# drprojects/superpoint_transformer

Measured on AMD Instinct MI355X. Metric: Mpoints/s SPT fwd+bwd on S3DIS-scale NAG, higher is better.
Workload: dtype f32 (the reference's shipped matmul class - configs/train.yaml:60-61 `float32_matmul_precision: high` = TF32 / bf16x3 next to `precision: 32` - as bf16x3: matrix products on the bf16 pipe with split operands, attention and the backward of the fused layers and of the attention blocks' Linears hi*hi +

## Files before the change

### superpoint_transformer_amd/csrc/fused_pool.hip

```cpp
#include <math.h>

#include <type_traits>

#include "common.hpp"

namespace spt {
namespace fpool {

typedef float f32x4 __attribute__((ext_vector_type(4)));
typedef __bf16 bf16x8 __attribute__((ext_vector_type(8)));
typedef __bf16 bf16x4 __attribute__((ext_vector_type(4)));
typedef short s16x4 __attribute__((ext_vector_type(4)));
#ifndef SPT_FPOOL_SKIP
#define SPT_FPOOL_SKIP 0
#endif
#ifndef SPT_FPOOL_WPAD
#define SPT_FPOOL_WPAD 16
#endif
constexpr int TR = 16;
constexpr int NWF = 8;
constexpr int ARG_NONE = 0x7fffffff;

__device__ __forceinline__ double xg_sum_d(double v) {
  v += __shfl_xor(v, 16, 64);
  v += __shfl_xor(v, 32, 64);
  return v;
}
__device__ __forceinline__ float xg_sum_f(float v) {
  v += __shfl_xor(v, 16, 64);
  v += __shfl_xor(v, 32, 64);
  return v;
}
__device__ __forceinline__ void wave_sync_lds() {
  __builtin_amdgcn_fence(__ATOMIC_RELEASE, "wavefront");
  __builtin_amdgcn_wave_barrier();
  __builtin_amdgcn_fence(__ATOMIC_ACQUIRE, "wavefront");
}
template <bool B16>
__device__ __forceinline__ float4 ld4(const float* __restrict__ base, int64_t elem) {
  if constexpr (B16) {
    const uint2 u = *reinterpret_cast<const uint2*>(reinterpret_cast<const uint16_t*>(base) + elem);
    return make_float4(__uint_as_float(u.x << 16), __uint_as_float(u.x & 0xffff0000u),
                       __uint_as_float(u.y << 16), __uint_as_float(u.y & 0xffff0000u));
  } else {
    return *reinterpret_cast<const float4*>(base + elem);
  }
}
template <int NV, typename V>
__device__ __forceinline__ void split2(const float (&x)[NV], V& hi, V& lo) {
#pragma unroll
  for (int i = 0; i < NV; ++i) {
    const __bf16 h = (__bf16)x[i];
    hi[i] = h;
    lo[i] = (__bf16)(x[i] - (float)h);
  }
}
template <int NV, typename V>
__device__ __forceinline__ void split3(const float (&x)[NV], V& h, V& m, V& l) {
#pragma unroll
  for (int i = 0; i < NV; ++i) {
    const __bf16 a = (__bf16)x[i];
    const float r1 = x[i] - (float)a;
    const __bf16 b = (__bf16)r1;
    const float r2 = r1 - (float)b;
    h[i] = a;
    m[i] = b;
    l[i] = (__bf16)r2;
  }
}
__device__ __forceinline__ f32x4 mfma16(const bf16x4& a, const bf16x4& b, f32x4 c) {
  return __builtin_amdgcn_mfma_f32_16x16x16bf16_1k(__builtin_bit_cast(s16x4, a),
                                                   __builtin_bit_cast(s16x4, b), c, 0, 0, 0);
}

template <bool X16>
struct RowChunk { typedef float4 type; };
template <>
struct RowChunk<true> { typedef uint2 type; };
template <bool X16>
__device__ __forceinline__ float4 widen(const typename RowChunk<X16>::type& u) {
  if constexpr (X16) {
    return make_float4(__uint_as_float(u.x << 16), __uint_as_float(u.x & 0xffff0000u),
                       __uint_as_float(u.y << 16), __uint_as_float(u.y & 0xffff0000u));
  } else {
    return u;
  }
}
template <int K, bool X16>
__device__ __forceinline__ void load_rows(const float* __restrict__ x, int rid_l,
                                          typename RowChunk<X16>::type (&v)[TR * (K / 4) / 64], int lane) {
  constexpr int CH = K / 4, NIT = TR * CH / 64;
  static_assert(TR * CH % 64 == 0, "whole waves of chunks");
#pragma unroll
  for (int j = 0; j < NIT; ++j) {
    const int q = lane + 64 * j, rr = q / CH, k = (q - rr * CH) << 2;
    const int64_t xr = (int64_t)__shfl(rid_l, rr, 64);
    if constexpr (X16)
      v[j] = *reinterpret_cast<const uint2*>(reinterpret_cast<const uint16_t*>(x) + xr * K + k);
    else
      v[j] = *reinterpret_cast<const float4*>(x + xr * K + k);
  }
}
template <int K, int LD, bool PRE, bool X16>
__device__ __forceinline__ void store_rows(const typename RowChunk<X16>::type (&v)[TR * (K / 4) / 64],
                                           int cnt, const float* tab, float slope, float* lds, int lane) {
  constexpr int CH = K / 4, NIT = TR * CH / 64;
#pragma unroll
  for (int j = 0; j < NIT; ++j) {
    const int q = lane + 64 * j, rr = q / CH, k = (q - rr * CH) << 2;
    float4 w = widen<X16>(v[j]);
    if constexpr (PRE) {
      const float4 a = *reinterpret_cast<const float4*>(tab + k);
      const float4 s = *reinterpret_cast<const float4*>(tab + K + k);
      const float4 b = *reinterpret_cast<const float4*>(tab + 2 * K + k);
      w.x = fmaf(w.x - a.x, s.x, b.x); w.y = fmaf(w.y - a.y, s.y, b.y);
      w.z = fmaf(w.z - a.z, s.z, b.z); w.w = fmaf(w.w - a.w, s.w, b.w);
      w.x = w.x > 0.f ? w.x : w.x * slope; w.y = w.y > 0.f ? w.y : w.y * slope;
      w.z = w.z > 0.f ? w.z : w.z * slope; w.w = w.w > 0.f ? w.w : w.w * slope;
    }
    if (rr >= cnt) w = make_float4(0.f, 0.f, 0.f, 0.f);
    *reinterpret_cast<float4*>(lds + rr * LD + k) = w;
  }
}

__device__ __forceinline__ int64_t cut_at(int64_t p, int64_t r0, int64_t r1,
                                          const int32_t* __restrict__ pos_seg,
                                          const int32_t* __restrict__ rowptr) {
  if (p <= r0) return r0;
  if (p >= r1) return r1;
  const int s = __builtin_amdgcn_readfirstlane(pos_seg[p]);
  const int64_t b = (int64_t)__builtin_amdgcn_readfirstlane(rowptr[s]);
  if (b == p) return p;
  const int64_t e = (int64_t)__builtin_amdgcn_readfirstlane(rowptr[s + 1]);
  return e < r1 ? e : r1;
}

template <int K, int N, int PREC, bool IN16>
__global__ __launch_bounds__(NWF * 64, 2) void fwd_pool_kernel(
    const float* __restrict__ x, const int32_t* __restrict__ perm,
    const int32_t* __restrict__ pos_seg, const int32_t* __restrict__ rowptr,
    const float* __restrict__ W, const float* __restrict__ gnw, const float* __restrict__ pam,
    const float* __restrict__ psc, const float* __restrict__ pbs, float pslope,
    float* __restrict__ raw, int32_t* __restrict__ argpos, double* __restrict__ partial, FmlpRuns rt) {
  constexpr int KS = K / 32, KB = K / 16, NBK = N / 16, LDA = K + 4;
  constexpr int LDW = K + SPT_FPOOL_WPAD;
  static_assert(LDW % 32 == 16 || SPT_FPOOL_WPAD != 16, "conflict-free B fragments");
  constexpr int NPL = PREC == 3 ? 3 : (PREC == 2 ? 2 : 1);
  constexpr int NGB = KB * (KB + 1) / 2;
  constexpr int GLEN = K * K + K + 1;
  static_assert(K % 32 == 0 && N % 16 == 0, "shape");
  __shared__ __attribute__((aligned(16))) float a_lds[NWF][TR * LDA];
  __shared__ __attribute__((aligned(16))) float tab[4 * K];
  __shared__ __attribute__((aligned(16))) float sgn_l[N];
  __shared__ __attribute__((aligned(16))) __bf16 wpl[NPL][N * LDW];
  __shared__ double gred[K * K + K];
  const int lane = threadIdx.x & 63;
  const int wid = __builtin_amdgcn_readfirstlane(threadIdx.x >> 6);
  const int g = lane >> 4, c = lane & 15;
  const int run = blockIdx.y, gph = rt.g[run];
  const int64_t r0 = rt.r0[run], r1 = rt.r1[run];
  pam += (size_t)gph * K;
  psc += (size_t)gph * K;
  partial += ((size_t)run * gridDim.x + blockIdx.x) * GLEN;
  float* al = a_lds[wid];
  for (int i = threadIdx.x; i < K; i += NWF * 64) {
    tab[i] = pam[i];
    tab[K + i] = psc[i];
    tab[2 * K + i] = pbs[i];
    const float bsv = pbs[i];
    tab[3 * K + i] = PREC == 1 ? 0.f : (bsv > 0.f ? bsv : pslope * bsv);
  }
  for (int i = threadIdx.x; i < N; i += NWF * 64) sgn_l[i] = gnw[i] < 0.f ? -1.f : 1.f;
  for (int i = threadIdx.x; i < N * K; i += NWF * 64) {
    const int n = i / K, k = i - n * K;
    const float w = gnw[n] < 0.f ? -W[i] : W[i];
    if constexpr (PREC == 3) {
      const float w1[1] = {w};
      __bf16 a[1], b[1], cc[1];
      split3<1>(w1, a, b, cc);
      wpl[0][n * LDW + k] = a[0];
      wpl[1][n * LDW + k] = b[0];
      wpl[2][n * LDW + k] = cc[0];
    } else if constexpr (PREC == 2) {
      const __bf16 hh = (__bf16)w;
      wpl[0][n * LDW + k] = hh;
      wpl[1][n * LDW + k] = (__bf16)(w - (float)hh);
    } else {
      wpl[0][n * LDW + k] = (__bf16)w;
    }
  }
  __syncthreads();

  f32x4 GA[NGB];
#pragma unroll
  for (int i = 0; i < NGB; ++i) GA[i] = (f32x4){0.f, 0.f, 0.f, 0.f};
  float sy[KB];
#pragma unroll
  for (int kb = 0; kb < KB; ++kb) sy[kb] = 0.f;
  float pm[NBK];
  int pp[NBK];
#pragma unroll
  for (int nb = 0; nb < NBK; ++nb) {
    pm[nb] = -INFINITY;
    pp[nb] = ARG_NONE;
  }
  int cur_seg = -1;
  auto flush = [&](int seg) {
#pragma unroll
    for (int nb = 0; nb < NBK; ++nb) {
      float m = pm[nb];
      int a = pp[nb];
#pragma unroll
      for (int off = 16; off <= 32; off <<= 1) {
        const float om = __shfl_xor(m, off, 64);
        const int oa = __shfl_xor(a, off, 64);
        const bool t = (om > m) || (om == m && oa < a);
        m = t ? om : m;
        a = t ? oa : a;
      }
      if ((nb & 3) == g) {
        const size_t o = (size_t)seg * N + 16 * nb + c;
        raw[o] = m * sgn_l[16 * nb + c];
        argpos[o] = a;
      }
      pm[nb] = -INFINITY;
      pp[nb] = ARG_NONE;
    }
  };

  const int64_t nw = (int64_t)gridDim.x * NWF, w = (int64_t)blockIdx.x * NWF + wid;
  const int64_t per = (((r1 - r0 + nw - 1) / nw) + TR - 1) / TR * TR;
  const int64_t pa0 = cut_at(r0 + w * per, r0, r1, pos_seg, rowptr);
  const int64_t pb0 = (w == nw - 1) ? r1 : cut_at(r0 + (w + 1) * per, r0, r1, pos_seg, rowptr);
  const bool has_rows = pa0 < pb0;
  const int64_t plast = pb0 - 1;
  auto ids_of = [&](int64_t p, int& rid, int& sg) {
    int64_t q = p + (lane & (TR - 1));
    q = q < plast ? q : plast;
    rid = perm ? perm[q] : (int)q;
    sg = pos_seg[q];
  };
  if (has_rows) {
  int seg_a, seg_b, rid_c, seg_c;
  typename RowChunk<IN16>::type xv[TR * (K / 4) / 64];
  {
    int rid0, rid1;
    ids_of(pa0, rid0, seg_a);
    load_rows<K, IN16>(x, rid0, xv, lane);
    ids_of(pa0 + TR, rid1, seg_b);
    ids_of(pa0 + 2 * TR, rid_c, seg_c);
    wave_sync_lds();
    store_rows<K, LDA, true, IN16>(xv, (int)((pb0 - pa0) < TR ? (pb0 - pa0) : TR), tab, pslope, al, lane);
    load_rows<K, IN16>(x, rid1, xv, lane);
  }
  for (int64_t p = pa0; p < pb0; p += TR) {
    const int cnt = (int)((pb0 - p) < TR ? (pb0 - p) : TR);
    wave_sync_lds();
    f32x4 C[NBK];
#pragma unroll
    for (int nb = 0; nb < NBK; ++nb) C[nb] = (f32x4){0.f, 0.f, 0.f, 0.f};
    if constexpr (!(SPT_FPOOL_SKIP & 4)) {
      constexpr int NSTEP = KS * NBK;
      constexpr int LA = NPL == 3 ? 2 : (NPL == 2 ? 3 : 6);
      bf16x8 wf[LA + 1][NPL];
      auto ldw = [&](int step, bf16x8 (&w)[NPL]) {
        const int ks = step / NBK, nb = step - ks * NBK;
        const int wo = (16 * nb + c) * LDW + 32 * ks + 8 * g;
#pragma unroll
        for (int pl = 0; pl < NPL; ++pl) w[pl] = *reinterpret_cast<const bf16x8*>(&wpl[pl][wo]);
      };
#pragma unroll
      for (int i = 0; i < LA; ++i) ldw(i, wf[i]);
      bf16x8 x1, x2, x3;
#pragma unroll
      for (int step = 0; step < NSTEP; ++step) {
        const int ks = step / NBK, nb = step - ks * NBK;
        if (nb == 0) {
          const float4 a0 = *reinterpret_cast<const float4*>(al + c * LDA + 32 * ks + 8 * g);
          const float4 a1 = *reinterpret_cast<const float4*>(al + c * LDA + 32 * ks + 8 * g + 4);
          const float av[8] = {a0.x, a0.y, a0.z, a0.w, a1.x, a1.y, a1.z, a1.w};
          if constexpr (PREC == 3) {
            split3<8>(av, x1, x2, x3);
          } else if constexpr (PREC == 2) {
            split2<8>(av, x1, x2);
          } else {
#pragma unroll
            for (int i = 0; i < 8; ++i) x1[i] = (__bf16)av[i];
          }
        }
        if (step + LA < NSTEP) ldw(step + LA, wf[(step + LA) % (LA + 1)]);
        __builtin_amdgcn_sched_barrier(0);
        const bf16x8 (&w)[NPL] = wf[step % (LA + 1)];
        f32x4 acc = C[nb];
        if constexpr (PREC == 3) {
          acc = __builtin_amdgcn_mfma_f32_16x16x32_bf16(x3, w[0], acc, 0, 0, 0);
          acc = __builtin_amdgcn_mfma_f32_16x16x32_bf16(x1, w[NPL - 1], acc, 0, 0, 0);
          acc = __builtin_amdgcn_mfma_f32_16x16x32_bf16(x2, w[NPL > 1 ? 1 : 0], acc, 0, 0, 0);
          acc = __builtin_amdgcn_mfma_f32_16x16x32_bf16(x2, w[0], acc, 0, 0, 0);
          acc = __builtin_amdgcn_mfma_f32_16x16x32_bf16(x1, w[NPL > 1 ? 1 : 0], acc, 0, 0, 0);
        } else if constexpr (PREC == 2) {
          acc = __builtin_amdgcn_mfma_f32_16x16x32_bf16(x2, w[0], acc, 0, 0, 0);
          acc = __builtin_amdgcn_mfma_f32_16x16x32_bf16(x1, w[NPL - 1], acc, 0, 0, 0);
        }
        acc = __builtin_amdgcn_mfma_f32_16x16x32_bf16(x1, w[0], acc, 0, 0, 0);
        C[nb] = acc;
        __builtin_amdgcn_sched_barrier(0);
      }
    }
    if constexpr (!(SPT_FPOOL_SKIP & 1)) {
      bf16x4 Yh[KB], Yl[KB];
#pragma unroll
      for (int kb = 0; kb < KB; ++kb) {
        float yv[4];
#pragma unroll
        for (int r = 0; r < 4; ++r) yv[r] = al[(4 * g + r) * LDA + 16 * kb + c];
        if constexpr (PREC != 1) {
          const float sh = tab[3 * K + 16 * kb + c];
#pragma unroll
          for (int r = 0; r < 4; ++r) yv[r] = (4 * g + r < cnt) ? yv[r] - sh : 0.f;
        }
        if constexpr (PREC == 1) {
#pragma unroll
          for (int r = 0; r < 4; ++r) {
            Yh[kb][r] = (__bf16)yv[r];
            yv[r] = (float)Yh[kb][r];
          }
        } else {
          split2<4>(yv, Yh[kb], Yl[kb]);
        }
        sy[kb] += (yv[0] + yv[1]) + (yv[2] + yv[3]);
      }
      int gi = 0;
#pragma unroll
      for (int mi = 0; mi < KB; ++mi)
#pragma unroll
        for (int ni = mi; ni < KB; ++ni) {
          f32x4 acc = GA[gi];
          if constexpr (PREC != 1) {
            acc = mfma16(Yl[mi], Yl[ni], acc);
            acc = mfma16(Yl[mi], Yh[ni], acc);
            acc = mfma16(Yh[mi], Yl[ni], acc);
          }
          GA[gi] = mfma16(Yh[mi], Yh[ni], acc);
          ++gi;
        }
    }
    wave_sync_lds();
    {
      const int64_t left = pb0 - (p + TR);
      store_rows<K, LDA, true, IN16>(xv, (int)(left < 0 ? 0 : (left < TR ? left : TR)), tab, pslope, al, lane);
      asm volatile("" : "+v"(rid_c), "+v"(seg_c));
    }
    const int seg_cur = seg_a;
    if constexpr (!(SPT_FPOOL_SKIP & 2)) {
      const int pos0 = (int)p + 4 * g;
      int row = 0;
      while (row < cnt) {
        const int s = __builtin_amdgcn_readlane(seg_cur, row);
        const uint64_t diff = __ballot(lane < cnt && lane > row && seg_cur != s);
        const int e = diff ? (int)__builtin_ctzll(diff) : cnt;
        if (s != cur_seg) {
          if (cur_seg >= 0) flush(cur_seg);
          cur_seg = s;
        }
        if (row == 0 && e == TR) {
#pragma unroll
          for (int r = 0; r < 4; ++r)
#pragma unroll
            for (int nb = 0; nb < NBK; ++nb) {
              const float v = C[nb][r];
              const bool win = v > pm[nb];
              pm[nb] = win ? v : pm[nb];
              pp[nb] = win ? pos0 + r : pp[nb];
            }
        } else {
#pragma unroll
          for (int r = 0; r < 4; ++r) {
            const int rr = 4 * g + r;
            const bool in = rr >= row && rr < e;
#pragma unroll
            for (int nb = 0; nb < NBK; ++nb) {
              const float v = in ? C[nb][r] : -INFINITY;
              const bool win = v > pm[nb];
              pm[nb] = win ? v : pm[nb];
              pp[nb] = win ? pos0 + r : pp[nb];
            }
          }
        }
        row = e;
      }
    }
    load_rows<K, IN16>(x, rid_c, xv, lane);
    seg_a = seg_b;
    seg_b = seg_c;
    ids_of(p + 3 * TR, rid_c, seg_c);
  }
  }
  if (cur_seg >= 0) flush(cur_seg);

  for (int i = threadIdx.x; i < K * K + K; i += NWF * 64) gred[i] = 0.0;
  __syncthreads();
  for (int ww = 0; ww < NWF; ++ww) {
    if (wid == ww) {
      int gi = 0;
#pragma unroll
      for (int mi = 0; mi < KB; ++mi)
#pragma unroll
        for (int ni = mi; ni < KB; ++ni) {
#pragma unroll
          for (int r = 0; r < 4; ++r)
            gred[(16 * mi + 4 * g + r) * K + 16 * ni + c] += (double)GA[gi][r];
          ++gi;
        }
#pragma unroll
      for (int kb = 0; kb < KB; ++kb) {
        const double t = xg_sum_d((double)sy[kb]);
        if (g == 0) gred[K * K + 16 * kb + c] += t;
      }
    }
    __syncthreads();
  }
  const int64_t wfirst = (int64_t)blockIdx.x * NWF, wlast = wfirst + NWF - 1;
  const int64_t ba = cut_at(r0 + wfirst * per, r0, r1, pos_seg, rowptr);
  const int64_t bb = (wlast >= nw - 1) ? r1 : cut_at(r0 + (wlast + 1) * per, r0, r1, pos_seg, rowptr);
  const double nblk = (double)(bb > ba ? bb - ba : 0);
  for (int i = threadIdx.x; i < K * K; i += NWF * 64) {
    const int rr = i / K, cc = i - rr * K;
    const double gp = (rr / 16 <= cc / 16) ? gred[i] : gred[cc * K + rr];
    const double sr = (double)tab[3 * K + rr], sc_ = (double)tab[3 * K + cc];
    partial[i] = gp + sr * gred[K * K + cc] + gred[K * K + rr] * sc_ + nblk * sr * sc_;
  }
  for (int i = threadIdx.x; i < K; i += NWF * 64)
    partial[K * K + i] = gred[K * K + i] + nblk * (double)tab[3 * K + i];
  if (threadIdx.x == 0) partial[K * K + K] = (blockIdx.x == 0) ? (double)(r1 - r0) : 0.0;
}

template <int K>
__global__ __launch_bounds__(256) void gram_tables_kernel(
    const double* __restrict__ gram, const float* __restrict__ W, int N, int bfw,
    const float* __restrict__ weight, const float* __restrict__ mean_scale, float eps,
    double* __restrict__ total, float* __restrict__ mean, float* __restrict__ rstd,
    float* __restrict__ am, float* __restrict__ scale) {
  constexpr int GLEN = K * K + K + 1, CPB = 256 / K;
  __shared__ double gl[K * K + K];
  __shared__ double wl[CPB][K];
  __shared__ double r1[CPB][K], r2[CPB][K];
  const int b = blockIdx.y;
  const double* gr = gram + (size_t)b * GLEN;
  for (int i = threadIdx.x; i < K * K + K; i += 256) gl[i] = gr[i];
  const int cl = threadIdx.x / K, j = threadIdx.x - cl * K;
  const int c = blockIdx.x * CPB + cl;
  {
    float w = c < N ? W[(size_t)c * K + j] : 0.f;
    if (bfw) w = (float)(__bf16)w;
    wl[cl][j] = (double)w;
  }
  __syncthreads();
  double t = 0.0;
#pragma unroll 8
  for (int k = 0; k < K; ++k) t += gl[j * K + k] * wl[cl][k];
  r2[cl][j] = wl[cl][j] * t;
  r1[cl][j] = wl[cl][j] * gl[K * K + j];
  __syncthreads();
  for (int st = K / 2; st > 0; st >>= 1) {
    if (j < st) {
      r1[cl][j] += r1[cl][j + st];
      r2[cl][j] += r2[cl][j + st];
    }
    __syncthreads();
  }
  if (j != 0 || c >= N) return;
  double n = gr[K * K + K];
  const double nraw = n;
  if (n < 1.0) n = 1.0;
  const double s1 = r1[cl][0];
  double s2 = r2[cl][0];
  if (s2 < 0.0) s2 = 0.0;
  if (total) {
    double* tr = total + (size_t)b * (2 * N + 1);
    tr[c] = s1;
    tr[N + c] = s2;
    if (c == 0) tr[2 * N] = nraw;
  }
  const double mu = s1 / n;
  const double a = (double)mean_scale[c];
  double var = s2 / n - (2.0 * a - a * a) * mu * mu;
  if (var < 0.0) var = 0.0;
  const double rs = 1.0 / sqrt(var + (double)eps);
  const float mu32 = (float)mu, rs32 = (float)rs;
  const int o = b * N + c;
  mean[o] = mu32;
  rstd[o] = rs32;
  am[o] = (float)(a * (double)mu32);
  scale[o] = (float)((double)weight[c] * (double)rs32);
}

template <int K, bool IN16>
__global__ __launch_bounds__(256) void pool_apply_kernel(
    const int32_t* __restrict__ rowptr, const int32_t* __restrict__ perm,
    const int64_t* __restrict__ seg_graph, int64_t num_seg, int N, int64_t n_rows,
    const float* __restrict__ am, const float* __restrict__ sc, const float* __restrict__ bs,
    float slope, const float* __restrict__ gnw, const float* __restrict__ x,
    const float* __restrict__ W, const float* __restrict__ pam, const float* __restrict__ psc,
    const float* __restrict__ pbs, float pslope, int bfw, float* __restrict__ raw,
    int32_t* __restrict__ argpos, int32_t* __restrict__ arg, float* __restrict__ out) {
  const int64_t t4 = ((int64_t)blockIdx.x * blockDim.x + threadIdx.x) * 4;
  if (t4 >= num_seg * N) return;
  const int64_t s = t4 / N;
  const int c0 = (int)(t4 - s * N);
  const int a0 = rowptr[s], a1 = rowptr[s + 1];
  if (a1 <= a0) {
    const int32_t nr = (int32_t)n_rows;
    *reinterpret_cast<float4*>(out + t4) = make_float4(0.f, 0.f, 0.f, 0.f);
    *reinterpret_cast<float4*>(raw + t4) = make_float4(0.f, 0.f, 0.f, 0.f);
    if (arg) *reinterpret_cast<int4*>(arg + t4) = make_int4(nr, nr, nr, nr);
    *reinterpret_cast<int4*>(argpos + t4) = make_int4(nr, nr, nr, nr);
    return;
  }
  const int64_t gph = seg_graph ? seg_graph[s] : 0;
  const float4 h4 = *reinterpret_cast<const float4*>(raw + t4);
  const int4 p4 = *reinterpret_cast<const int4*>(argpos + t4);
  const float4 w4 = *reinterpret_cast<const float4*>(gnw + c0);
  const float4 am4 = *reinterpret_cast<const float4*>(am + gph * N + c0);
  const float4 sc4 = *reinterpret_cast<const float4*>(sc + gph * N + c0);
  const float4 bs4 = *reinterpret_cast<const float4*>(bs + c0);
  float hh[4] = {h4.x, h4.y, h4.z, h4.w};
  int pp[4] = {p4.x, p4.y, p4.z, p4.w};
  const float gw[4] = {w4.x, w4.y, w4.z, w4.w};
  const float aa[4] = {am4.x, am4.y, am4.z, am4.w}, ss[4] = {sc4.x, sc4.y, sc4.z, sc4.w};
  const float bb[4] = {bs4.x, bs4.y, bs4.z, bs4.w};
  float yy[4];
  int ar[4];
#pragma unroll
  for (int e = 0; e < 4; ++e) {
    if (gw[e] == 0.f) {
      const int c = c0 + e;
      pp[e] = a0;
      const int row = perm ? perm[a0] : a0;
      double acc = 0.0;
      for (int k = 0; k < K; ++k) {
        float v = IN16 ? __uint_as_float((unsigned)reinterpret_cast<const uint16_t*>(x)[(int64_t)row * K + k] << 16)
                       : x[(int64_t)row * K + k];
        v = fmaf(v - pam[gph * K + k], psc[gph * K + k], pbs[k]);
        v = v > 0.f ? v : v * pslope;
        float w = W[(size_t)c * K + k];
        if (bfw) {
          w = (float)(__bf16)w;
          v = (float)(__bf16)v;
        }
        acc += (double)v * (double)w;
      }
      hh[e] = (float)acc;
      raw[t4 + e] = hh[e];
      argpos[t4 + e] = pp[e];
    }
    if (arg) ar[e] = (pp[e] >= a0 && pp[e] < a1) ? (perm ? perm[pp[e]] : pp[e]) : (int32_t)n_rows;
    float y = fmaf(hh[e] - aa[e], ss[e], bb[e]);
    yy[e] = y > 0.f ? y : y * slope;
  }
  if (arg) *reinterpret_cast<int4*>(arg + t4) = make_int4(ar[0], ar[1], ar[2], ar[3]);
  *reinterpret_cast<float4*>(out + t4) = make_float4(yy[0], yy[1], yy[2], yy[3]);
}

__global__ __launch_bounds__(256) void pool_bwd_gm_kernel(
    const float* __restrict__ gout, const float* __restrict__ raw,
    const int64_t* __restrict__ seg_graph, int64_t num_seg, int N, const float* __restrict__ am,
    const float* __restrict__ sc, const float* __restrict__ bs, float slope,
    const float* __restrict__ c1, float* __restrict__ gm) {
  const int64_t t4 = ((int64_t)blockIdx.x * blockDim.x + threadIdx.x) * 4;
  if (t4 >= num_seg * N) return;
  const int64_t s = t4 / N;
  const int c = (int)(t4 - s * N);
  const int64_t gph = seg_graph ? seg_graph[s] : 0;
  const float4 go = *reinterpret_cast<const float4*>(gout + t4);
  const float4 hv = *reinterpret_cast<const float4*>(raw + t4);
  const float4 a = *reinterpret_cast<const float4*>(am + gph * N + c);
  const float4 sv = *reinterpret_cast<const float4*>(sc + gph * N + c);
  const float4 b = *reinterpret_cast<const float4*>(bs + c);
  const float4 k1 = *reinterpret_cast<const float4*>(c1 + gph * N + c);
  const float gg[4] = {go.x, go.y, go.z, go.w}, hh[4] = {hv.x, hv.y, hv.z, hv.w};
  const float aa[4] = {a.x, a.y, a.z, a.w}, ss[4] = {sv.x, sv.y, sv.z, sv.w};
  const float bb[4] = {b.x, b.y, b.z, b.w}, q1[4] = {k1.x, k1.y, k1.z, k1.w};
  float o[4];
#pragma unroll
  for (int e = 0; e < 4; ++e) {
    float g_ = gg[e];
    if (slope != 1.f) {
      const float y = fmaf(hh[e] - aa[e], ss[e], bb[e]);
      g_ = (y > 0.f) ? g_ : g_ * slope;
    }
    o[e] = q1[e] * g_;
  }
  *reinterpret_cast<float4*>(gm + t4) = make_float4(o[0], o[1], o[2], o[3]);
}

template <int K>
__global__ __launch_bounds__(256) void pool_bwd_coef_kernel(
    const float* __restrict__ W, int N, const float* __restrict__ am, const float* __restrict__ c2,
    const float* __restrict__ c3, float* __restrict__ M, float* __restrict__ c0) {
  const int b = blockIdx.x;
  extern __shared__ float sm[];
  float* Bc = sm;
  float* Ac = sm + N;
  for (int i = threadIdx.x; i < N; i += blockDim.x) {
    const float k2 = c2[b * N + i];
    Bc[i] = -k2;
    Ac[i] = fmaf(k2, am[b * N + i], -c3[b * N + i]);
  }
  __syncthreads();
  for (int i = blockIdx.y * blockDim.x + threadIdx.x; i < K * K + K; i += gridDim.y * blockDim.x) {
    double acc = 0.0;
    if (i < K * K) {
      const int j = i / K, k = i - j * K;
      for (int c = 0; c < N; ++c)
        acc += (double)W[(size_t)c * K + j] * (double)Bc[c] * (double)W[(size_t)c * K + k];
      M[(size_t)b * K * K + i] = (float)acc;
    } else {
      const int k = i - K * K;
      for (int c = 0; c < N; ++c) acc += (double)Ac[c] * (double)W[(size_t)c * K + k];
      c0[(size_t)b * K + k] = (float)acc;
    }
  }
}

template <int K>
__global__ __launch_bounds__(256) void pool_bwd_gw_dense_kernel(
    const double* __restrict__ gram, int B, const float* __restrict__ W, int N, int bfw,
    const float* __restrict__ am, const float* __restrict__ c2, const float* __restrict__ c3,
    float* __restrict__ gW) {
  constexpr int GLEN = K * K + K + 1;
  const int t = blockIdx.x * blockDim.x + threadIdx.x;
  if (t >= N * K) return;
  const int c = t / K, k = t - c * K;
  double acc = 0.0;
  for (int b = 0; b < B; ++b) {
    const double* gr = gram + (size_t)b * GLEN;
    const double k2 = (double)c2[b * N + c];
    const double Ac = (double)fmaf(c2[b * N + c], am[b * N + c], -c3[b * N + c]);
    double t1 = 0.0;
    for (int j = 0; j < K; ++j) {
      float w = W[(size_t)c * K + j];
      if (bfw) w = (float)(__bf16)w;
      t1 += (double)w * gr[j * K + k];
    }
    acc += -k2 * t1 + Ac * gr[K * K + k];
  }
  gW[t] = (float)((double)gW[t] + acc);
}

typedef __attribute__((address_space(3))) s16x4 lds_s16x4;
typedef __attribute__((address_space(3))) volatile int lds_flag_t;
__device__ __forceinline__ void flag_set(lds_flag_t* f, int v) {
  asm volatile("s_waitcnt lgkmcnt(0)" ::: "memory");
  *f = v;
}
__device__ __forceinline__ bool flag_wait(lds_flag_t* f, int v) {
  int spins = 0;
  bool ok = true;
#pragma clang loop unroll(disable)
  while (__builtin_amdgcn_readfirstlane(*f) < v) {
    __builtin_amdgcn_s_sleep(1);
    if (++spins > (1 << 22)) {
      ok = false;
      break;
    }
  }
  asm volatile("" ::: "memory");
  return ok;
}
template <int C>
__device__ __forceinline__ int pl_off(int row, int col) {
  constexpr int RPL = 128 / C;
  static_assert(C == 32 || C == 64 || C == 128, "plane row of 64, 128 or 256 bytes");
  const int swz = ((row / RPL) & (8 / RPL - 1)) << 1;
  return row * C + ((((col >> 3) ^ swz) << 3) | (col & 7));
}
__device__ __forceinline__ s16x4 tr_read(const __bf16* p) {
  return __builtin_amdgcn_ds_read_tr16_b64_v4i16((lds_s16x4*)(__attribute__((address_space(3))) void*)p);
}
template <int K, int N, bool LO, bool X16, int NW>
__global__ __launch_bounds__(NW * 64, NW / 4) void bwd_pool_kernel(
    const float* __restrict__ gm, const int32_t* __restrict__ argpos,
    const int32_t* __restrict__ perm, const int32_t* __restrict__ pos_seg,
    const float* __restrict__ xprev, const float* __restrict__ pam,
    const float* __restrict__ psc, const float* __restrict__ pbs, float pslope,
    const float* __restrict__ W, const float* __restrict__ Mg, const float* __restrict__ c0g,
    float* __restrict__ gx, float* __restrict__ gw_partial, double* __restrict__ pstat_partial,
    FmlpRuns rt) {
  constexpr int KB = K / 16, NBK = N / 16, NS = N / 32, KS = K / 32;
  constexpr int NBH = NBK / 2, KBH = KB / 2;
  constexpr int LDX = K + 4;
  constexpr int LDT = N + SPT_FPOOL_WPAD, LDM = K + SPT_FPOOL_WPAD;
  static_assert((LDT % 32 == 16 && LDM % 32 == 16) || SPT_FPOOL_WPAD != 16, "conflict-free B fragments");
  static_assert(K % 32 == 0 && N % 64 == 0 && NW % 2 == 0, "shape");
  constexpr int NP = NW / 2, NPL = LO ? 2 : 1;
  constexpr int HR = TR / 2;
  constexpr int CH = K / 4, NIT = HR * CH / 64;
  static_assert(HR * CH % 64 == 0, "whole waves of chunks");
  constexpr int NH = N / 2;
  static_assert(NH <= 64 && (NH & (NH - 1)) == 0, "one channel per lane");
  constexpr int NZ = TR * (NH / 8) / 64;
  static_assert(TR * (NH / 8) % 64 == 0, "whole waves of chunks");
  constexpr int T_X = 0;
  constexpr int T_Y = T_X + TR * LDX * 4;
  constexpr int T_S = T_Y + NPL * TR * K * 2;
  constexpr int T_PAD = T_S + NPL * TR * N * 2;
  constexpr int T_FLAG = T_PAD + 16;
  constexpr int T_END = T_FLAG + 16;
  static_assert(T_Y % 16 == 0 && T_END % 16 == 0, "16-byte chunks");
  constexpr int F_STAGED = 0, F_DONE = 2;
  __shared__ __attribute__((aligned(16))) unsigned char tile_lds[NP * T_END];
  __shared__ __attribute__((aligned(16))) __bf16 wt_hi[K * LDT];
  __shared__ __attribute__((aligned(16))) __bf16 wt_lo[LO ? K * LDT : 8];
  __shared__ __attribute__((aligned(16))) __bf16 mt_hi[K * LDM];
  __shared__ __attribute__((aligned(16))) __bf16 mt_lo[LO ? K * LDM : 8];
  __shared__ __attribute__((aligned(16))) float pt[3 * K];
  __shared__ __attribute__((aligned(16))) float c0l[K];
  const int lane = threadIdx.x & 63;
  const int wid = __builtin_amdgcn_readfirstlane(threadIdx.x >> 6);
  const int hf = wid & 1;
  const int nb0 = hf * NBH, kb0 = hf * KBH;
  const int g = lane >> 4, c = lane & 15;
  const int run = blockIdx.y, gph = rt.g[run];
  const int64_t r0 = rt.r0[run], r1 = rt.r1[run];
  pam += (size_t)gph * K;
  psc += (size_t)gph * K;
  Mg += (size_t)gph * K * K;
  c0g += (size_t)gph * K;
  constexpr int SCR = 4 * (K / 32) * 64;
  float* gw_scratch = gw_partial + (size_t)gridDim.y * gridDim.x * N * K +
                      (size_t)run * gridDim.x * (NW / 2) * 2 * SCR;
  gw_partial += (size_t)run * gridDim.x * N * K;
  pstat_partial += (size_t)run * gridDim.x * (NW / 2) * (2 * K + 1);
  unsigned char* tl = tile_lds + (wid >> 1) * T_END;
  float* xr = reinterpret_cast<float*>(tl + T_X);
  __bf16* yp = reinterpret_cast<__bf16*>(tl + T_Y);
  __bf16* sp = reinterpret_cast<__bf16*>(tl + T_S);
  __bf16* pad = reinterpret_cast<__bf16*>(tl + T_PAD);
  lds_flag_t* flg = (lds_flag_t*)(__attribute__((address_space(3))) void*)(tl + T_FLAG);
  for (int i = threadIdx.x; i < K * N; i += NW * 64) {
    const int k = i / N, n = i - k * N;
    const float w = W[(size_t)n * K + k];
    const __bf16 hh = (__bf16)w;
    wt_hi[k * LDT + n] = hh;
    if constexpr (LO) wt_lo[k * LDT + n] = (__bf16)(w - (float)hh);
  }
  for (int i = threadIdx.x; i < K * K; i += NW * 64) {
    const int k = i / K, j = i - k * K;
    const float m = Mg[(size_t)j * K + k];
    const __bf16 hh = (__bf16)m;
    mt_hi[k * LDM + j] = hh;
    if constexpr (LO) mt_lo[k * LDM + j] = (__bf16)(m - (float)hh);
  }
  for (int i = threadIdx.x; i < K; i += NW * 64) {
    pt[i] = pam[i];
    pt[K + i] = psc[i];
    pt[2 * K + i] = pbs[i];
    c0l[i] = c0g[i];
  }
  if (lane < 4) flg[lane] = 0;
  __syncthreads();

  f32x4 C3[NBH][KB];
#pragma unroll
  for (int nb = 0; nb < NBH; ++nb)
#pragma unroll
    for (int kb = 0; kb < KB; ++kb) C3[nb][kb] = (f32x4){0.f, 0.f, 0.f, 0.f};
  double p1[KBH], p2[KBH];
#pragma unroll
  for (int kb = 0; kb < KBH; ++kb) p1[kb] = p2[kb] = 0.0;

  const int64_t ntiles = (r1 - r0 + TR - 1) / TR;
  const int64_t pair = (int64_t)blockIdx.x * (NW / 2) + (wid >> 1);
  const int64_t npairs = (int64_t)gridDim.x * (NW / 2);
  auto cnt_of = [&](int64_t t) {
    const int64_t row0 = r0 + t * TR;
    return (t < ntiles) ? (int)((r1 - row0) < TR ? (r1 - row0) : TR) : 0;
  };
  auto load_ids = [&](int64_t t, int& rid, int& sg) {
    const int64_t tt = t < ntiles ? t : ntiles - 1;
    int64_t q = r0 + tt * TR + (lane & (TR - 1));
    q = q < r1 - 1 ? q : r1 - 1;
    rid = perm ? perm[q] : (int)q;
    sg = pos_seg[q];
  };
  auto load_half = [&](int rid, typename RowChunk<X16>::type (&v)[NIT]) {
#pragma unroll
    for (int j = 0; j < NIT; ++j) {
      const int q = lane + 64 * j, rl = q / CH, k = (q - rl * CH) << 2;
      const int64_t xrow = (int64_t)__shfl(rid, HR * hf + rl, 64);
      if constexpr (X16)
        v[j] = *reinterpret_cast<const uint2*>(reinterpret_cast<const uint16_t*>(xprev) + xrow * K + k);
      else
        v[j] = *reinterpret_cast<const float4*>(xprev + xrow * K + k);
    }
  };
  const int chn = hf * NH + (lane & (NH - 1));
  const bool sc_on = lane < NH;
  auto load_seg = [&](int sgm, int& ap, float& gv) {
    const size_t o = (size_t)sgm * N + chn;
    ap = argpos[o];
    gv = gm[o];
  };
  auto scatter = [&](int ap, float gv, int row0i, int lo, int hi) {
    const int rr = ap - row0i;
    const bool ok = sc_on && rr >= lo && rr < hi;
    const int o = pl_off<N>(rr & (TR - 1), chn);
    const __bf16 h = (__bf16)gv;
    *(ok ? sp + o : pad) = h;
    if constexpr (LO) *(ok ? sp + TR * N + o : pad + 1) = (__bf16)(gv - (float)h);
  };
  if (ntiles > 0) {
  int rid_l, seg_l, rid_n, seg_n;
  load_ids(pair, rid_l, seg_l);
  typename RowChunk<X16>::type xv[NIT];
  load_half(rid_l, xv);
  int apA, apB;
  float gvA, gvB;
  {
    const int c0 = cnt_of(pair < ntiles ? pair : ntiles - 1);
    load_seg(__builtin_amdgcn_readlane(seg_l, 0), apA, gvA);
    load_seg(__builtin_amdgcn_readlane(seg_l, c0 - 1), apB, gvB);
  }
  load_ids(pair + npairs, rid_n, seg_n);
  {
    float* scratch = gw_scratch + ((size_t)pair * 2 + hf) * SCR;
#pragma unroll
    for (int i = 0; i < 4 * KBH; ++i) scratch[lane + 64 * i] = 0.f;
  }
  int kseq = 0;
  bool lost = false;
  auto tile = [&](auto full_c, int64_t t) {
    constexpr bool FULL = decltype(full_c)::value;
    const int64_t row0 = r0 + t * TR;
    const int cnt = FULL ? TR : cnt_of(t);
    auto ynorm = [&](float v, int k, bool ok) {
      v = fmaf(v - pt[k], pt[K + k], pt[2 * K + k]);
      v = (v > 0.f) ? v : v * pslope;
      return ok ? v : 0.f;
    };
    if (!lost) lost = !flag_wait(flg + F_DONE + (hf ^ 1), kseq);
#pragma unroll
    for (int j = 0; j < NIT; ++j) {
      const int q = lane + 64 * j, rl = q / CH, k = (q - rl * CH) << 2, rr = HR * hf + rl;
      const bool ok = rr < cnt;
      float4 w = widen<X16>(xv[j]);
      if (!ok) w = make_float4(0.f, 0.f, 0.f, 0.f);
      *reinterpret_cast<float4*>(xr + rr * LDX + k) = w;
      const float yv[4] = {ynorm(w.x, k, ok), ynorm(w.y, k + 1, ok), ynorm(w.z, k + 2, ok),
                           ynorm(w.w, k + 3, ok)};
      bf16x4 yh, yl;
      const int o = pl_off<K>(rr, k);
      if constexpr (LO) {
        split2<4>(yv, yh, yl);
        *reinterpret_cast<bf16x4*>(yp + TR * K + o) = yl;
      } else {
#pragma unroll
        for (int i = 0; i < 4; ++i) yh[i] = (__bf16)yv[i];
      }
      *reinterpret_cast<bf16x4*>(yp + o) = yh;
    }
    {
#pragma unroll
      for (int j = 0; j < NZ; ++j) {
        const int q = lane + 64 * j, rr = q / (NH / 8), ch = hf * (NH / 8) + (q - rr * (NH / 8));
        const int o = pl_off<N>(rr, 8 * ch);
        const bf16x8 z = __builtin_bit_cast(bf16x8, make_uint4(0u, 0u, 0u, 0u));
        *reinterpret_cast<bf16x8*>(sp + o) = z;
        if constexpr (LO) *reinterpret_cast<bf16x8*>(sp + TR * N + o) = z;
      }
      const int sA = __builtin_amdgcn_readlane(seg_l, 0);
      const int sB = __builtin_amdgcn_readlane(seg_l, cnt - 1);
      const uint64_t notA = __ballot(lane < cnt && seg_l != sA);
      const int eA = notA ? (int)__builtin_ctzll(notA) : cnt;
      const uint64_t isB = __ballot(lane < cnt && seg_l == sB);
      const int bB = (int)__builtin_ctzll(isB);
      scatter(apA, gvA, (int)row0, 0, eA);
      if (sB != sA) scatter(apB, gvB, (int)row0, bB, cnt);
      int row = eA;
      while (row < bB) {
        const int sgm = __builtin_amdgcn_readlane(seg_l, row);
        const uint64_t diff = __ballot(lane < cnt && lane > row && seg_l != sgm);
        const int e = diff ? (int)__builtin_ctzll(diff) : cnt;
        int ap;
        float gv;
        load_seg(sgm, ap, gv);
        scatter(ap, gv, (int)row0, row, e);
        row = e;
      }
    }
    const int rid_cur = rid_l;
    load_half(rid_n, xv);
    {
      const int64_t tn = t + npairs < ntiles ? t + npairs : ntiles - 1;
      load_seg(__builtin_amdgcn_readlane(seg_n, 0), apA, gvA);
      load_seg(__builtin_amdgcn_readlane(seg_n, cnt_of(tn) - 1), apB, gvB);
    }
    rid_l = rid_n;
    seg_l = seg_n;
    load_ids(t + 2 * npairs, rid_n, seg_n);
    flag_set(flg + F_STAGED + hf, kseq + 1);
    if (!lost) lost = !flag_wait(flg + F_STAGED + (hf ^ 1), kseq + 1);
    if constexpr (!(SPT_FPOOL_SKIP & 8)) {
      const int trow = 4 * g + (c >> 2), tcol = 4 * (c & 3);
      s16x4 Xh[KB];
      bf16x8 Xc[LO ? KB : 1];
#pragma unroll
      for (int kb = 0; kb < KB; ++kb) {
        const __bf16* p = yp + pl_off<K>(trow, 16 * kb + tcol);
        Xh[kb] = tr_read(p);
        if constexpr (LO)
          Xc[kb] = __builtin_bit_cast(bf16x8, __builtin_shufflevector(Xh[kb], tr_read(p + TR * K),
                                                                      0, 1, 2, 3, 4, 5, 6, 7));
      }
#pragma unroll
      for (int nb = 0; nb < NBH; ++nb) {
        const __bf16* p = sp + pl_off<N>(trow, 16 * (nb0 + nb) + tcol);
        const s16x4 sh = tr_read(p);
        if constexpr (LO) {
          const s16x4 sl = tr_read(p + TR * N);
          const bf16x8 Sc = __builtin_bit_cast(bf16x8, __builtin_shufflevector(sl, sh, 0, 1, 2, 3, 4, 5, 6, 7));
#pragma unroll
          for (int kb = 0; kb < KB; ++kb) {
            const f32x4 acc = __builtin_amdgcn_mfma_f32_16x16x32_bf16(Sc, Xc[kb], C3[nb][kb], 0, 0, 0);
            C3[nb][kb] = __builtin_amdgcn_mfma_f32_16x16x16bf16_1k(sh, Xh[kb], acc, 0, 0, 0);
          }
        } else {
#pragma unroll
          for (int kb = 0; kb < KB; ++kb)
            C3[nb][kb] = __builtin_amdgcn_mfma_f32_16x16x16bf16_1k(sh, Xh[kb], C3[nb][kb], 0, 0, 0);
        }
      }
    }
    {
      f32x4 CX[KBH];
      float xo[4][KBH];
#pragma unroll
      for (int kb = 0; kb < KBH; ++kb) {
        const float z = c0l[16 * (kb0 + kb) + c];
        CX[kb] = (f32x4){z, z, z, z};
#pragma unroll
        for (int r = 0; r < 4; ++r) xo[r][kb] = xr[(4 * g + r) * LDX + 16 * (kb0 + kb) + c];
      }
      constexpr int NPLB = LO ? 2 : 1, LAB = 2;
      constexpr int NST1 = NS * KBH, NST = NST1 + KS * KBH;
      bf16x8 bf[LAB + 1][NPLB];
      auto ldb = [&](int step, bf16x8 (&b)[NPLB]) {
        if (step < NST1) {
          const int sg = step / KBH, kb = step - sg * KBH;
          const int wo = (16 * (kb0 + kb) + c) * LDT + 32 * sg + 8 * g;
          b[0] = *reinterpret_cast<const bf16x8*>(wt_hi + wo);
          if constexpr (LO) b[NPLB - 1] = *reinterpret_cast<const bf16x8*>(wt_lo + wo);
        } else {
          const int st = step - NST1, ks = st / KBH, kb = st - ks * KBH;
          const int mo = (16 * (kb0 + kb) + c) * LDM + 32 * ks + 8 * g;
          b[0] = *reinterpret_cast<const bf16x8*>(mt_hi + mo);
          if constexpr (LO) b[NPLB - 1] = *reinterpret_cast<const bf16x8*>(mt_lo + mo);
        }
      };
#pragma unroll
      for (int i = 0; i < LAB; ++i) ldb(i, bf[i]);
      bf16x8 ah, alo;
#pragma unroll
      for (int step = 0; step < ((SPT_FPOOL_SKIP & 16) ? 0 : NST); ++step) {
        const bool first = step < NST1;
        const int sub = first ? step : step - NST1;
        const int blk = sub / KBH, kb = sub - blk * KBH;
        if (kb == 0) {
          const __bf16* p = first ? sp + pl_off<N>(c, 32 * blk + 8 * g) : yp + pl_off<K>(c, 32 * blk + 8 * g);
          ah = *reinterpret_cast<const bf16x8*>(p);
          if constexpr (LO) alo = *reinterpret_cast<const bf16x8*>(p + (first ? TR * N : TR * K));
        }
        if (step + LAB < NST) ldb(step + LAB, bf[(step + LAB) % (LAB + 1)]);
        __builtin_amdgcn_sched_barrier(0);
        const bf16x8 (&b)[NPLB] = bf[step % (LAB + 1)];
        f32x4 acc = CX[kb];
        if constexpr (LO) {
          acc = __builtin_amdgcn_mfma_f32_16x16x32_bf16(alo, b[0], acc, 0, 0, 0);
          acc = __builtin_amdgcn_mfma_f32_16x16x32_bf16(ah, b[NPLB - 1], acc, 0, 0, 0);
        }
        CX[kb] = __builtin_amdgcn_mfma_f32_16x16x32_bf16(ah, b[0], acc, 0, 0, 0);
// ... 226 lines not shown
```

Before: 355.2.

## Stage pre-split bf16 Gram operands in LDS and use 16x16x32 MFMA

In the forward pool kernel, the centred activation rows are now split into bf16 hi/lo planes once, when they are stored to LDS. A swizzled layout lets the Gram loop fetch them with ds_read_tr16 transposed reads, where it used to read fp32 values, subtract the shift and split them per use. The four 16x16x16 MFMAs per Gram block become two 16x16x32 MFMAs that pack the lo*lo, lo*hi, hi*lo and hi*hi products together. The column sums move into the store step with double accumulators, and the Gram reduction buffer now aliases the tile LDS to save shared memory. This adds a __syncthreads before the reduction and makes the store step heavier.

```diff
diff --git a/superpoint_transformer_amd/csrc/fused_pool.hip b/superpoint_transformer_amd/csrc/fused_pool.hip
--- a/superpoint_transformer_amd/csrc/fused_pool.hip
+++ b/superpoint_transformer_amd/csrc/fused_pool.hip
@@ -68,9 +68,17 @@
     l[i] = (__bf16)r2;
   }
 }
-__device__ __forceinline__ f32x4 mfma16(const bf16x4& a, const bf16x4& b, f32x4 c) {
-  return __builtin_amdgcn_mfma_f32_16x16x16bf16_1k(__builtin_bit_cast(s16x4, a),
-                                                   __builtin_bit_cast(s16x4, b), c, 0, 0, 0);
+
+typedef __attribute__((address_space(3))) s16x4 lds_s16x4;
+template <int C>
+__device__ __forceinline__ int pl_off(int row, int col) {
+  constexpr int RPL = 128 / C;
+  static_assert(C == 32 || C == 64 || C == 128, "plane row of 64, 128 or 256 bytes");
+  const int swz = ((row / RPL) & (8 / RPL - 1)) << 1;
+  return row * C + ((((col >> 3) ^ swz) << 3) | (col & 7));
+}
+__device__ __forceinline__ s16x4 tr_read(const __bf16* p) {
+  return __builtin_amdgcn_ds_read_tr16_b64_v4i16((lds_s16x4*)(__attribute__((address_space(3))) void*)p);
 }
 
 template <bool X16>
@@ -101,10 +109,14 @@
       v[j] = *reinterpret_cast<const float4*>(x + xr * K + k);
   }
 }
-template <int K, int LD, bool PRE, bool X16>
+template <int K, int LD, bool PRE, bool X16, int GPL = 0>
 __device__ __forceinline__ void store_rows(const typename RowChunk<X16>::type (&v)[TR * (K / 4) / 64],
-                                           int cnt, const float* tab, float slope, float* lds, int lane) {
+                                           int cnt, const float* tab, float slope, float* lds, int lane,
+                                           __bf16* pl = nullptr, double* sy = nullptr) {
   constexpr int CH = K / 4, NIT = TR * CH / 64;
+  static_assert(GPL == 0 || 64 % CH == 0, "a lane keeps its columns from chunk to chunk");
+  const bool part = cnt < TR;
+  float ts[4] = {0.f, 0.f, 0.f, 0.f};
 #pragma unroll
   for (int j = 0; j < NIT; ++j) {
     const int q = lane + 64 * j, rr = q / CH, k = (q - rr * CH) << 2;
@@ -118,8 +130,39 @@
       w.x = w.x > 0.f ? w.x : w.x * slope; w.y = w.y > 0.f ? w.y : w.y * slope;
       w.z = w.z > 0.f ? w.z : w.z * slope; w.w = w.w > 0.f ? w.w : w.w * slope;
     }
-    if (rr >= cnt) w = make_float4(0.f, 0.f, 0.f, 0.f);
-    *reinterpret_cast<float4*>(lds + rr * LD + k) = w;
+    if constexpr (GPL == 0) {
+      if (rr >= cnt) w = make_float4(0.f, 0.f, 0.f, 0.f);
+      *reinterpret_cast<float4*>(lds + rr * LD + k) = w;
+    } else {
+      const float4 sh = *reinterpret_cast<const float4*>(tab + 3 * K + k);
+      float d[4] = {w.x - sh.x, w.y - sh.y, w.z - sh.z, w.w - sh.w};
+      if (part) {
+        if (rr >= cnt) {
+          w = make_float4(0.f, 0.f, 0.f, 0.f);
+          d[0] = d[1] = d[2] = d[3] = 0.f;
+        }
+      }
+      *reinterpret_cast<float4*>(lds + rr * LD + k) = w;
+      const int o = pl_off<K>(rr, k);
+      bf16x4 yh, yl;
+      if constexpr (GPL == 2) {
+        split2<4>(d, yh, yl);
+        *reinterpret_cast<bf16x4*>(pl + TR * K + o) = yl;
+      } else {
+#pragma unroll
+        for (int i = 0; i < 4; ++i) {
+          yh[i] = (__bf16)d[i];
+          d[i] = (float)yh[i];
+        }
+      }
+      *reinterpret_cast<bf16x4*>(pl + o) = yh;
+#pragma unroll
+      for (int i = 0; i < 4; ++i) ts[i] += d[i];
+    }
+  }
+  if constexpr (GPL != 0) {
+#pragma unroll
+    for (int i = 0; i < 4; ++i) sy[i] += (double)ts[i];
   }
 }
 
@@ -149,11 +192,15 @@
   constexpr int NGB = KB * (KB + 1) / 2;
   constexpr int GLEN = K * K + K + 1;
   static_assert(K % 32 == 0 && N % 16 == 0, "shape");
-  __shared__ __attribute__((aligned(16))) float a_lds[NWF][TR * LDA];
+  constexpr int GPL = PREC == 1 ? 1 : 2;
+  constexpr int T_Y = TR * LDA * 4, T_END = T_Y + GPL * TR * K * 2;
+  static_assert(T_Y % 16 == 0 && T_END % 16 == 0, "16-byte chunks");
+  static_assert((K * K + K) * 8 <= NWF * T_END, "the Gram reduction fits the tile records");
+  __shared__ __attribute__((aligned(16))) unsigned char tile_lds[NWF * T_END];
   __shared__ __attribute__((aligned(16))) float tab[4 * K];
   __shared__ __attribute__((aligned(16))) float sgn_l[N];
   __shared__ __attribute__((aligned(16))) __bf16 wpl[NPL][N * LDW];
-  __shared__ double gred[K * K + K];
+  double* gred = reinterpret_cast<double*>(tile_lds);
   const int lane = threadIdx.x & 63;
   const int wid = __builtin_amdgcn_readfirstlane(threadIdx.x >> 6);
   const int g = lane >> 4, c = lane & 15;
@@ -162,7 +209,8 @@
   pam += (size_t)gph * K;
   psc += (size_t)gph * K;
   partial += ((size_t)run * gridDim.x + blockIdx.x) * GLEN;
-  float* al = a_lds[wid];
+  float* al = reinterpret_cast<float*>(tile_lds + wid * T_END);
+  __bf16* yp = reinterpret_cast<__bf16*>(tile_lds + wid * T_END + T_Y);
   for (int i = threadIdx.x; i < K; i += NWF * 64) {
     tab[i] = pam[i];
     tab[K + i] = psc[i];
@@ -194,9 +242,7 @@
   f32x4 GA[NGB];
 #pragma unroll
   for (int i = 0; i < NGB; ++i) GA[i] = (f32x4){0.f, 0.f, 0.f, 0.f};
-  float sy[KB];
-#pragma unroll
-  for (int kb = 0; kb < KB; ++kb) sy[kb] = 0.f;
+  double sy[4] = {0.0, 0.0, 0.0, 0.0};
   float pm[NBK];
   int pp[NBK];
 #pragma unroll
@@ -250,7 +296,8 @@
     ids_of(pa0 + TR, rid1, seg_b);
     ids_of(pa0 + 2 * TR, rid_c, seg_c);
     wave_sync_lds();
-    store_rows<K, LDA, true, IN16>(xv, (int)((pb0 - pa0) < TR ? (pb0 - pa0) : TR), tab, pslope, al, lane);
+    store_rows<K, LDA, true, IN16, GPL>(xv, (int)((pb0 - pa0) < TR ? (pb0 - pa0) : TR), tab, pslope, al, lane,
+                                        yp, sy);
     load_rows<K, IN16>(x, rid1, xv, lane);
   }
   for (int64_t p = pa0; p < pb0; p += TR) {
@@ -308,47 +355,38 @@
       }
     }
     if constexpr (!(SPT_FPOOL_SKIP & 1)) {
-      bf16x4 Yh[KB], Yl[KB];
+      s16x4 Yh[KB];
+      bf16x8 LL[PREC != 1 ? KB : 1], HH[PREC != 1 ? KB : 1], LH[PREC != 1 ? KB : 1];
 #pragma unroll
       for (int kb = 0; kb < KB; ++kb) {
-        float yv[4];
-#pragma unroll
-        for (int r = 0; r < 4; ++r) yv[r] = al[(4 * g + r) * LDA + 16 * kb + c];
+        const __bf16* p = yp + pl_off<K>(4 * g + (c >> 2), 16 * kb + 4 * (c & 3));
+        Yh[kb] = tr_read(p);
         if constexpr (PREC != 1) {
-          const float sh = tab[3 * K + 16 * kb + c];
-#pragma unroll
-          for (int r = 0; r < 4; ++r) yv[r] = (4 * g + r < cnt) ? yv[r] - sh : 0.f;
-        }
-        if constexpr (PREC == 1) {
-#pragma unroll
-          for (int r = 0; r < 4; ++r) {
-            Yh[kb][r] = (__bf16)yv[r];
-            yv[r] = (float)Yh[kb][r];
+          const s16x4 Yl = tr_read(p + TR * K);
+          LL[kb] = __builtin_bit_cast(bf16x8, __builtin_shufflevector(Yl, Yl, 0, 1, 2, 3, 4, 5, 6, 7));
+          HH[kb] = __builtin_bit_cast(bf16x8, __builtin_shufflevector(Yh[kb], Yh[kb], 0, 1, 2, 3, 4, 5, 6, 7));
+          LH[kb] = __builtin_bit_cast(bf16x8, __builtin_shufflevector(Yl, Yh[kb], 0, 1, 2, 3, 4, 5, 6, 7));
+        }
+      }
+      int gi = 0;
+#pragma unroll
+      for (int mi = 0; mi < KB; ++mi)
+#pragma unroll
+        for (int ni = mi; ni < KB; ++ni) {
+          if constexpr (PREC != 1) {
+            const f32x4 acc = __builtin_amdgcn_mfma_f32_16x16x32_bf16(LL[mi], LH[ni], GA[gi], 0, 0, 0);
+            GA[gi] = __builtin_amdgcn_mfma_f32_16x16x32_bf16(HH[mi], LH[ni], acc, 0, 0, 0);
+          } else {
+            GA[gi] = __builtin_amdgcn_mfma_f32_16x16x16bf16_1k(Yh[mi], Yh[ni], GA[gi], 0, 0, 0);
           }
-        } else {
-          split2<4>(yv, Yh[kb], Yl[kb]);
-        }
-        sy[kb] += (yv[0] + yv[1]) + (yv[2] + yv[3]);
-      }
-      int gi = 0;
-#pragma unroll
-      for (int mi = 0; mi < KB; ++mi)
-#pragma unroll
-        for (int ni = mi; ni < KB; ++ni) {
-          f32x4 acc = GA[gi];
-          if constexpr (PREC != 1) {
-            acc = mfma16(Yl[mi], Yl[ni], acc);
-            acc = mfma16(Yl[mi], Yh[ni], acc);
-            acc = mfma16(Yh[mi], Yl[ni], acc);
-          }
-          GA[gi] = mfma16(Yh[mi], Yh[ni], acc);
           ++gi;
         }
     }
     wave_sync_lds();
     {
       const int64_t left = pb0 - (p + TR);
-      store_rows<K, LDA, true, IN16>(xv, (int)(left < 0 ? 0 : (left < TR ? left : TR)), tab, pslope, al, lane);
+      store_rows<K, LDA, true, IN16, GPL>(xv, (int)(left < 0 ? 0 : (left < TR ? left : TR)), tab, pslope, al,
+                                          lane, yp, sy);
       asm volatile("" : "+v"(rid_c), "+v"(seg_c));
     }
     const int seg_cur = seg_a;
@@ -398,6 +436,7 @@
   }
   if (cur_seg >= 0) flush(cur_seg);
 
+  __syncthreads();
   for (int i = threadIdx.x; i < K * K + K; i += NWF * 64) gred[i] = 0.0;
   __syncthreads();
   for (int ww = 0; ww < NWF; ++ww) {
@@ -413,9 +452,11 @@
           ++gi;
         }
 #pragma unroll
-      for (int kb = 0; kb < KB; ++kb) {
-        const double t = xg_sum_d((double)sy[kb]);
-        if (g == 0) gred[K * K + 16 * kb + c] += t;
+      for (int i = 0; i < 4; ++i) {
+        double t = sy[i];
+#pragma unroll
+        for (int off = K / 4; off < 64; off <<= 1) t += __shfl_xor(t, off, 64);
+        if (lane < K / 4) gred[K * K + 4 * lane + i] += t;
       }
     }
     __syncthreads();
@@ -648,7 +689,6 @@
   gW[t] = (float)((double)gW[t] + acc);
 }
 
-typedef __attribute__((address_space(3))) s16x4 lds_s16x4;
 typedef __attribute__((address_space(3))) volatile int lds_flag_t;
 __device__ __forceinline__ void flag_set(lds_flag_t* f, int v) {
   asm volatile("s_waitcnt lgkmcnt(0)" ::: "memory");
@@ -667,16 +707,6 @@
   }
   asm volatile("" ::: "memory");
   return ok;
-}
-template <int C>
-__device__ __forceinline__ int pl_off(int row, int col) {
-  constexpr int RPL = 128 / C;
-  static_assert(C == 32 || C == 64 || C == 128, "plane row of 64, 128 or 256 bytes");
-  const int swz = ((row / RPL) & (8 / RPL - 1)) << 1;
-  return row * C + ((((col >> 3) ^ swz) << 3) | (col & 7));
-}
-__device__ __forceinline__ s16x4 tr_read(const __bf16* p) {
-  return __builtin_amdgcn_ds_read_tr16_b64_v4i16((lds_s16x4*)(__attribute__((address_space(3))) void*)p);
 }
 template <int K, int N, bool LO, bool X16, int NW>
 __global__ __launch_bounds__(NW * 64, NW / 4) void bwd_pool_kernel(
```

Result: no change. 356.7 (median of 3 runs) (+0.4%).
